# radjkarl/imgProcessor

Hardware: AMD Instinct MI355X
Metric: Mpix/s undistort+5x5 filter, 4K f32 (higher is better)
Workload: dtype f32

## Files before the change

imgprocessor_amd/csrc/fused_sep_c.hip:

```cpp
#include "fused_sep_impl.hpp"

int ipa_fused_sep_launch_c(ipa_ctx* ctx, const ipa::FusedCall& f, const ipa::FusedSep& q) {
  return ipa::fused_sep_k<1>(ctx, f, q);
}

template <typename T> static int strip_remap_int_launch(ipa_ctx* ctx, const ipa::FusedCall& f) {
  using namespace ipa;
  using Src = SampleRowSrc<T, kLinear, MapCoord>;
  FusedCall part[2];
  const SharedPlan plan = fused_plan(ctx, sep_shared<Src, 1>::value && IPA_PIPE_EDGE, f, part);
  if (plan == kPerFrameLoop) return 1;
  if (plan == kSharedLoop) part[0] = f;
  const int parts = plan == kSharedSplit ? 2 : 1;
  for (int i = 0; i < parts; i++) {
    WaveParams p = part[i].p;
    sep_grid<Src, 1>(ctx, p, part[i].n_frames);
    if (!p.frames_wg) return 1;
  }
  Src s;
  fused_source(s, f, f.map);
  s.q5 = 1;
  s.ccval = 0.f;
  const double one = 1.0;
  for (int i = 0; i < parts; i++) {
    s.src = part[i].src;
    const int rc = launch_sep<Src, 1, T>(ctx, part[i].p, s, &one, &one, part[i].n_frames, 0.f);
    if (rc) return rc;
  }
  return IPA_OK;
}
int ipa_fused_sep_launch_c16(ipa_ctx* ctx, const ipa::FusedCall& f) { return strip_remap_int_launch<uint16_t>(ctx, f); }
int ipa_fused_sep_launch_c8(ipa_ctx* ctx, const ipa::FusedCall& f) { return strip_remap_int_launch<uint8_t>(ctx, f); }
```

imgprocessor_amd/csrc/wave_pipe.hpp:

```cpp
#pragma once

namespace ipa {

typedef int v4i __attribute__((ext_vector_type(4)));

#ifndef IPA_PIPE
#define IPA_PIPE 1
#endif
#ifndef IPA_PIPE_ROWS
#define IPA_PIPE_ROWS 4
#endif
#ifndef IPA_PIPE_REUSE
#define IPA_PIPE_REUSE 1
#endif
#ifndef IPA_PIPE_STAY
#define IPA_PIPE_STAY 0
#endif
#ifndef IPA_SHARE_TAPS
#define IPA_SHARE_TAPS 0
#endif
#ifndef IPA_DEBUG_HALO_LEVEL
#define IPA_DEBUG_HALO_LEVEL 0
#endif
#ifndef IPA_LANE_NATURAL
// ... 84 lines not shown
}
__device__ __forceinline__ void pipe_store1(unsigned x, unsigned voff, uint8_t* sbase) {
  asm volatile(IPA_SGPR_HAZARD "global_store_dword %0, %1, %2 " IPA_STORE_FLAVOUR "\n\ts_nop 0" ::"v"(voff), "v"(x), "s"(sbase));
}
__device__ __forceinline__ unsigned cv16_round(float v) {
  float r = rintf(v);
  r = r > 0.f ? r : 0.f;
  r = r < 65535.f ? r : 65535.f;
  return (unsigned)r;
}
__device__ __forceinline__ void pipe_gather2(float& a, float& b, unsigned off, v4i rs) {
#ifdef IPA_DEBUG_NO_GATHER
  a = __uint_as_float(off | 0x3f000000u);
  b = a;
  return;
#endif
#ifdef IPA_DEBUG_ONE_DWORD
  asm volatile(IPA_SGPR_HAZARD "buffer_load_dword %0, %1, %2, 0 offen" : "=v"(a) : "v"(off), "s"(rs));
  b = a;
  return;
#endif
  asm volatile(IPA_SGPR_HAZARD "buffer_load_dword %0, %2, %3, 0 offen\n\t"
               "buffer_load_dword %1, %2, %3, 0 offen offset:4"
               : "=v"(a), "=v"(b)
               : "v"(off), "s"(rs));
}
__device__ __forceinline__ void pipe_gather1(float& a, unsigned off, v4i rs) {
  asm volatile(IPA_SGPR_HAZARD "buffer_load_dword %0, %1, %2, 0 offen" : "=v"(a) : "v"(off), "s"(rs));
}
__device__ __forceinline__ void pipe_gather1_b16(float& a, unsigned off, v4i rs) {
  asm volatile(IPA_SGPR_HAZARD "buffer_load_ushort %0, %1, %2, 0 offen" : "=v"(a) : "v"(off), "s"(rs));
}
__device__ __forceinline__ void pipe_gather1_b16_masked(float& a, unsigned off, v4i rs, unsigned long long m) {
  unsigned long long sv;
  asm volatile(IPA_SGPR_HAZARD "s_mov_b64 %1, exec\n\t"
               "s_mov_b64 exec, %4\n\t"
               "buffer_load_ushort %0, %2, %3, 0 offen\n\t"
               "s_mov_b64 exec, %1"
               : "+v"(a), "=&s"(sv)
               : "v"(off), "s"(rs), "s"(m));
}
__device__ __forceinline__ void pipe_gather1_masked(float& a, unsigned off, v4i rs,
                                                    unsigned long long m) {
  unsigned long long sv;
  asm volatile(IPA_SGPR_HAZARD "s_mov_b64 %1, exec\n\t"
               "s_mov_b64 exec, %4\n\t"
               "buffer_load_dword %0, %2, %3, 0 offen\n\t"
// ... 391 lines not shown
    else vm_wait<kTapOps>();
    pin_map(m);
    footprint(m, txnn, tynn, offnn, interiornn);
    issue_map(m, t + 3);
  };

  float txc[NS], tyc[NS];
  unsigned offc[NS], inc = (1u << NS) - 1u;
  int tb = 0;
#pragma unroll 1
  do {
    if (tb + 0 < T) step(tb + 0, ga, gb, txa, tya, offa, ina, txb, tyb, offb, inb, txc, tyc, offc, inc);
    if (tb + 1 < T) step(tb + 1, gb, ga, txb, tyb, offb, inb, txc, tyc, offc, inc, txa, tya, offa, ina);
    if (tb + 2 < T) step(tb + 2, ga, gb, txc, tyc, offc, inc, txa, tya, offa, ina, txb, tyb, offb, inb);
    if (tb + 3 < T) step(tb + 3, gb, ga, txa, tya, offa, ina, txb, tyb, offb, inb, txc, tyc, offc, inc);
    if (tb + 4 < T) step(tb + 4, ga, gb, txb, tyb, offb, inb, txc, tyc, offc, inc, txa, tya, offa, ina);
    if (tb + 5 < T) step(tb + 5, gb, ga, txc, tyc, offc, inc, txa, tya, offa, ina, txb, tyb, offb, inb);
    tb += 6;
  } while (tb < T);
#undef hoff
}

template <bool HALO> struct ring_row { static constexpr int value = HALO ? 832 + 128 : 832; };

template <int K> struct DenseFilter {
  static constexpr int kTaps = K;
  const Weights<float, K * K>& wts;
  unsigned lane4_opaque;
  v2f acc[K][2];
  __device__ __forceinline__ DenseFilter(const Weights<float, K * K>& w) : wts(w) {
    lane4_opaque = 4u * (threadIdx.x & 63u);
    asm volatile("" : "+v"(lane4_opaque));
  }
  template <bool EDGE> __device__ __forceinline__ v4f row(const float* xp, unsigned lane, const Cols&) {
    return pipe_filter_row<K>(wts, xp, lane, lane4_opaque, acc);
  }
};

template <int K, int QM, bool EDGE, bool HALO, typename Filter, typename ST, typename Coord, bool CV16 = false>
__device__ __forceinline__ void wave_run_strip_shared(const WaveParams& p,
                                                      const SampleRowSrc<ST, kLinear, Coord>& src,
                                                      Filter& filt, float* xp, float* ring,
                                                      unsigned wave, const Cols& c, int y0,
                                                      int nrows, bool writer, float* dst) {
  using G = wave_geom<K, HALO>;
  using C = typename Coord::coord_t;
  constexpr int NS = 4;
  constexpr int NSP = HALO ? 5 : 4;
  constexpr int HP = 2 * G::H;
  static_assert(!HALO || HP <= 8, "at most 8 halo pixels (32 halo lanes, 128 record floats)");
  constexpr int RR = ring_row<HALO>::value;
  constexpr bool kTable = coord_is_table<Coord>::value;
  constexpr int NR = sizeof(ST) == 4 ? 2 : 1;
  constexpr int SH = sizeof(ST) == 4 ? 2 : (sizeof(ST) == 2 ? 1 : 0);
  constexpr bool kU8 = sizeof(ST) == 1;
  constexpr bool FIX8 = kU8 && CV16;
  static_assert(std::is_same<ST, float>::value || std::is_same<ST, uint16_t>::value || std::is_same<ST, uint8_t>::value,
                "float32 / uint16 / uint8 frames");
  constexpr int W = IPA_WPB;
  constexpr bool NAT = IPA_LANE_NATURAL != 0 && !HALO;
  constexpr int R = 2 * W;
  constexpr int kMapOps = kTable ? 2 * NSP : 0;
  static_assert(W == 2 || W == 4 || W == 8, "steps of a block alternate the tap-register roles");
  const int T = nrows + K - 1;
  const unsigned lane = threadIdx.x & 63u;
  constexpr unsigned CB = sizeof(C);
  const unsigned voff = 16u * lane, moff = NAT ? 4u * CB * lane : CB * lane;
  auto ucol = [&](int k) -> int { return NAT ? c.uu[k] : c.uq[k]; };
  auto pxcol = [&](int k) -> int { return NAT ? 4 * (int)lane + k : (int)lane + 64 * k; };
  static_assert(!CV16 || (K == 1 && QM == 1 && !HALO && sizeof(ST) <= 2), "CV16: integer frames, 1/32-px coordinates, no filter");
  float* outs = dst + ((long)y0 * p.dpitch + c.xs);
  uint16_t* outs16 = reinterpret_cast<uint16_t*>(dst) + ((long)y0 * p.dpitch + c.xs);
  uint8_t* outs8 = reinterpret_cast<uint8_t*>(dst) + ((long)y0 * p.dpitch + c.xs);
  const int yb = y0 - G::H;
  const C* mxr = nullptr;
  const C* myr = nullptr;
  if constexpr (kTable) {
    mxr = src.coord.mx + (EDGE ? 0 : (long)yb * src.coord.pitch + c.xs);
    myr = src.coord.my + (EDGE ? 0 : (long)yb * src.coord.pitch + c.xs);
  }
  auto row_of = [&](int t) -> int {
    if constexpr (EDGE) return resolve_idx(yb + t, p.dh, p.cby);
    else return yb + t;
  };
  const SrcView& s = src.s;
  const unsigned long long fb = (unsigned long long)src.fbase;
  const v4i rs = v4i{(int)(unsigned)fb, (int)((unsigned)(fb >> 32) & 0xffffu), (int)src.src_bytes,
                     0x00020000};
  const unsigned pitch_b = (unsigned)s.pitch << SH;
  float* rlane = ring + 4u * lane;
  const unsigned hcol = halo_pos<G::H>(lane);
  const unsigned long long pmask = (1ull << HP) - 1ull;
  const unsigned long long qmask = (1ull << (4 * HP)) - 1ull;
  const unsigned hq = lane < 4u * HP ? lane >> 2 : (unsigned)HP - 1u;
  const unsigned hpos = kRowPad - G::H + halo_pos<G::H>(hq);
  int uhq = 0;
  if constexpr (HALO && EDGE) uhq = resolve_idx(c.xs - G::H + (int)halo_pos<G::H>(hq), p.dw, p.cbx);
  constexpr unsigned kHTapIn = 1u, kHAnyIn = 2u, kHSlow = 4u, kHInterior = 8u;

  C pm[2 * NSP] = {};
  auto issue_coords = [&](int r) {
    if constexpr (kTable) {
      if constexpr (EDGE) {
        const int rr = row_of(r < T ? r : T - 1);
        const long o = (long)(rr < 0 ? 0 : rr) * src.coord.pitch;
#pragma unroll
        for (int k = 0; k < 4; k++) pipe_load1<0>(pm[k], CB * (unsigned)(ucol(k) < 0 ? 0 : ucol(k)), mxr + o);
        if constexpr (HALO) pipe_load1_masked<0>(pm[4], CB * (unsigned)(c.uh < 0 ? 0 : c.uh), mxr + o, pmask);
#pragma unroll
        for (int k = 0; k < 4; k++) pipe_load1<0>(pm[NSP + k], CB * (unsigned)(ucol(k) < 0 ? 0 : ucol(k)), myr + o);
        if constexpr (HALO) pipe_load1_masked<0>(pm[NSP + 4], CB * (unsigned)(c.uh < 0 ? 0 : c.uh), myr + o, pmask);
      } else {
        const long o = (long)(r < T ? r : T - 1) * src.coord.pitch;
        static_for<0, 4>([&](auto Kk) {
          constexpr int k = decltype(Kk)::value;
          pipe_load1<(NAT ? 1 : 64) * (int)CB * k>(pm[k], moff, mxr + o);
        });
        if constexpr (HALO) pipe_load1_masked<0>(pm[4], CB * hcol, mxr + o - G::H, pmask);
        static_for<0, 4>([&](auto Kk) {
          constexpr int k = decltype(Kk)::value;
          pipe_load1<(NAT ? 1 : 64) * (int)CB * k>(pm[NSP + k], moff, myr + o);
        });
        if constexpr (HALO) pipe_load1_masked<0>(pm[NSP + 4], CB * hcol, myr + o - G::H, pmask);
      }
    }
  };
  auto publish = [&](int r) {
    C sx[NSP], sy[NSP];
    if constexpr (kTable) {
#pragma unroll
      for (int k = 0; k < 2 * NSP; k++) vm_pin(pm[k]);
#pragma unroll
      for (int k = 0; k < NSP; k++) { sx[k] = pm[k]; sy[k] = pm[NSP + k]; }
    } else {
      const int rc = r < T ? r : T - 1;
      const int rr = row_of(rc);
#pragma unroll
      for (int k = 0; k < 4; k++) {
        if constexpr (EDGE) src.coord.get(ucol(k) < 0 ? 0 : ucol(k), rr < 0 ? 0 : rr, sx[k], sy[k]);
        else src.coord.get(c.xs + pxcol(k), rr, sx[k], sy[k]);
      }
      if constexpr (HALO) {
        if constexpr (EDGE) src.coord.get(c.uh < 0 ? 0 : c.uh, rr < 0 ? 0 : rr, sx[4], sy[4]);
        else src.coord.get(c.xs - G::H + (int)(lane < (unsigned)HP ? hcol : (unsigned)G::H), rr, sx[4], sy[4]);
      }
    }
    float tx[NSP], ty[NSP];
    int e[NSP];
    unsigned interior;
    batch_footprint_linear<NSP, QM>(s, sx, sy, tx, ty, e, interior);
    if constexpr (HALO) interior |= lane < (unsigned)HP ? 0u : 0x10u;
    if (s.border == IPA_BORDER_CONSTANT && __builtin_amdgcn_ballot_w64(interior != (1u << NSP) - 1u))
      interior |= border_tap_bits<NSP, QM, NR == 1, C>(s, sx, sy, interior);
    float* slot = rlane + (unsigned)(r % R) * RR;
    *reinterpret_cast<v4i*>(slot) = v4i{e[0] << SH, e[1] << SH, e[2] << SH, e[3] << SH};
    *reinterpret_cast<v4f*>(slot + 256) = v4f{tx[0], tx[1], tx[2], tx[3]};
    *reinterpret_cast<v4f*>(slot + 512) = v4f{ty[0], ty[1], ty[2], ty[3]};
    float* rowp = ring + (unsigned)(r % R) * RR;
    reinterpret_cast<unsigned*>(rowp + 768)[lane] = interior & ~0x0f000010u;
    if constexpr (HALO) {
      if (lane < (unsigned)HP) {
        const bool in4 = (interior >> 4) & 1u;
        const unsigned vb = (interior >> 24) & 15u;
        const bool slow = !in4 && (s.border != IPA_BORDER_CONSTANT || (interior & kBorderSlow) != 0u);
        float* hrow = rowp + 832 + 16u * lane;
#pragma unroll
        for (int tap = 0; tap < 4; tap++) {
          const unsigned o = ((unsigned)e[4] << SH) + (NR == 2 ? (unsigned)(tap & 1) * 4u : 0u) +
                             (unsigned)(tap >> 1) * pitch_b;
          const unsigned fl = ((in4 || ((vb >> tap) & 1u)) ? kHTapIn : 0u) | ((in4 || vb) ? kHAnyIn : 0u) |
                              (slow ? kHSlow : 0u) | (in4 ? kHInterior : 0u);
          *reinterpret_cast<v4f*>(hrow + 4 * tap) = v4f{__uint_as_float(o), tx[4], ty[4], __uint_as_float(fl)};
        }
      }
    }
  };
  auto footprint = [&](int r, float (&tx)[NS], float (&ty)[NS], unsigned (&off)[NS],
                       unsigned& interior) {
    const float* slot = rlane + (unsigned)(r % R) * RR;
    const float* rowp = ring + (unsigned)(r % R) * RR;
    const v4i qo = *reinterpret_cast<const v4i*>(slot);
    const v4f qx = *reinterpret_cast<const v4f*>(slot + 256), qy = *reinterpret_cast<const v4f*>(slot + 512);
    interior = reinterpret_cast<const unsigned*>(rowp + 768)[lane];
    off[0] = (unsigned)qo.x; off[1] = (unsigned)qo.y; off[2] = (unsigned)qo.z; off[3] = (unsigned)qo.w;
    tx[0] = qx.x; tx[1] = qx.y; tx[2] = qx.z; tx[3] = qx.w;
    ty[0] = qy.x; ty[1] = qy.y; ty[2] = qy.z; ty[3] = qy.w;
  };
  auto halo_record = [&](int r, unsigned& off, float& tx, float& ty, unsigned& fl) {
    const float* rowp = ring + (unsigned)(r % R) * RR;
    const v4f q = *reinterpret_cast<const v4f*>(rowp + 832 + 4u * (lane < 4u * HP ? lane : 4u * HP - 1u));
    off = __float_as_uint(q.x); tx = q.y; ty = q.z; fl = __float_as_uint(q.w);
  };
  auto gather = [&](float (&g)[NS * NR], int k, unsigned o) {
#if IPA_SHARE_TAPS == 9
    if constexpr (NR == 2) { pipe_gather1(g[2 * k], o, rs); return; }
#endif
    if constexpr (NR == 2) pipe_gather2(g[2 * k], g[2 * k + 1], o, rs);
    else if constexpr (kU8) pipe_gather1_b16(g[k], o, rs);
    else pipe_gather1(g[k], o, rs);
  };
  auto gather_masked = [&](float (&g)[NS * NR], int k, unsigned o, unsigned long long m) {
#if IPA_SHARE_TAPS == 9
    if constexpr (NR == 2) { pipe_gather1_masked(g[2 * k], o, rs, m); return; }
#endif
    if constexpr (NR == 2) pipe_gather2_masked(g[2 * k], g[2 * k + 1], o, rs, m);
    else if constexpr (kU8) pipe_gather1_b16_masked(g[k], o, rs, m);
    else pipe_gather1_masked(g[k], o, rs, m);
// ... 11 lines not shown
#if IPA_SHARE_TAPS == 9
    if constexpr (NR == 2) { v0 = g[2 * k]; v1 = from_lane_above(v0); return; }
#endif
    if constexpr (NR == 2) { v0 = g[2 * k]; v1 = g[2 * k + 1]; }
    else if constexpr (kU8) { v0 = (float)(__float_as_uint(g[k]) & 0xffu); v1 = (float)((__float_as_uint(g[k]) >> 8) & 0xffu); }
    else TapLoad<uint16_t, float>::unpack(__float_as_uint(g[k]), v0, v1);
  };

  float ga[NS * NR] = {}, gb[NS * NR] = {};
  float txa[NS], tya[NS], txb[NS], tyb[NS];
  unsigned offa[NS], offb[NS], ina, inb;
  float hga = 0.f, hgb = 0.f, htxa = 0.f, htya = 0.f, htxb = 0.f, htyb = 0.f;
  unsigned hfla = 0u, hflb = 0u;

#ifdef IPA_DEBUG_STAMPS
  unsigned stamp_acc[8] = {0, 0, 0, 0, 0, 0, 0, 0};
  unsigned stamp_prev = 0;
#define IPA_STAMP0() stamp_prev = (unsigned)__builtin_amdgcn_s_memtime()
#define IPA_STAMP(i) { const unsigned now_ = (unsigned)__builtin_amdgcn_s_memtime(); stamp_acc[i] += now_ - stamp_prev; stamp_prev = now_; }
#else
#define IPA_STAMP0()
#define IPA_STAMP(i)
#endif
  issue_coords((int)wave);
  vm_wait<0>();
  publish((int)wave);
  asm volatile("s_waitcnt lgkmcnt(0)\n\ts_barrier" ::: "memory");
  issue_coords(W + (int)wave);
  footprint(0, txa, tya, offa, ina);
  gather_row(ga, offa, 0u);
  gather_row(gb, offa, pitch_b);
  if constexpr (HALO && IPA_DEBUG_HALO_LEVEL < 2) {
    unsigned ho;
    halo_record(0, ho, htxa, htya, hfla);
    if (IPA_DEBUG_HALO_LEVEL < 1) pipe_gather1_masked(hga, ho, rs, qmask);
  }

  auto step = [&](auto St, int t, float (&top)[NS * NR], float (&bot)[NS * NR], const float (&tx)[NS],
                  const float (&ty)[NS], const unsigned (&off)[NS], unsigned interior,
                  float (&txn)[NS], float (&tyn)[NS], unsigned (&offn)[NS], unsigned& interiorn,
                  float& hg, float htx, float hty, unsigned hfl,
                  float& hgn, float& htxn, float& htyn, unsigned& hfln) {
    constexpr int STEP = decltype(St)::value;
    IPA_STAMP0();
    if constexpr (STEP == W - 1) {
#ifndef IPA_DEBUG_NO_BARRIER
      asm volatile("s_waitcnt lgkmcnt(0)\n\ts_barrier" ::: "memory");
#endif
      IPA_STAMP(0);
      issue_coords(t + 1 + W + (int)wave);
    }
    const bool stored = t >= K && t <= T;
    if constexpr (STEP == W - 1) {
      if (stored) vm_wait<kMapOps + 1>();
      else vm_wait<kMapOps>();
    } else {
      if (stored) vm_wait<1>();
      else vm_wait<0>();
    }
    pin_taps(top);
    pin_taps(bot);
    IPA_STAMP(1);
    if constexpr (HALO && IPA_DEBUG_HALO_LEVEL < 1) vm_pin(hg);
    if constexpr (STEP == W - 2) publish(t + 2 + (int)wave);
    float cur[NS];
#pragma unroll
    for (int k = 0; k < NS; k++) {
      const float wx0 = 1.f - tx[k], wx1 = tx[k], wy0 = 1.f - ty[k], wy1 = ty[k];
      float v00, v01, v10, v11;
      taps_of(top, k, v00, v01);
      taps_of(bot, k, v10, v11);
      if constexpr (FIX8) {
        cur[k] = fix8_sum((int)v00, (int)v01, (int)v10, (int)v11, tx[k], ty[k]);
      } else if constexpr (CV16) {
        cur[k] = cv16_sum(v00, v01, v10, v11, wx0, wx1, wy0, wy1);
      } else {
        float r0 = wx0 * v00;
        r0 = ipa_fma(wx1, v01, r0);
        float o = wy0 * r0;
        float r1 = wx0 * v10;
        r1 = ipa_fma(wx1, v11, r1);
        cur[k] = ipa_fma(wy1, r1, o);
      }
    }
    int rowt = 0;
    if constexpr (EDGE) {
      rowt = row_of(t < T ? t : T - 1);
#pragma unroll
      for (int k = 0; k < 4; k++) cur[k] = (rowt < 0 || ucol(k) < 0) ? src.ccval : cur[k];
    }
    if constexpr (NAT) {
      *reinterpret_cast<v4f*>(xp + kRowPad + 4u * lane) = v4f{cur[0], cur[1], cur[2], cur[3]};
    } else {
#pragma unroll
      for (int k = 0; k < 4; k++) xp[kRowPad + 64u * k + lane] = cur[k];
    }
    if constexpr (HALO && IPA_DEBUG_HALO_LEVEL < 2) {
      float v = hg;
      if constexpr (NR == 1) {
        float lo, hi;
        TapLoad<uint16_t, float>::unpack(__float_as_uint(hg), lo, hi);
        v = (lane & 1u) ? hi : lo;
      }
      v = (hfl & kHTapIn) ? v : src.cval;
      const int vi = __float_as_int(v);
      const float v00 = __int_as_float(__builtin_amdgcn_update_dpp(vi, vi, 0x00, 0xf, 0xf, false));
      const float v01 = __int_as_float(__builtin_amdgcn_update_dpp(vi, vi, 0x55, 0xf, 0xf, false));
      const float v10 = __int_as_float(__builtin_amdgcn_update_dpp(vi, vi, 0xaa, 0xf, 0xf, false));
      const float v11 = __int_as_float(__builtin_amdgcn_update_dpp(vi, vi, 0xff, 0xf, 0xf, false));
      const float wx0 = 1.f - htx, wx1 = htx, wy0 = 1.f - hty, wy1 = hty;
      float r0 = wx0 * v00;
      r0 = ipa_fma(wx1, v01, r0);
// ... 18 lines not shown
      if (__builtin_amdgcn_ballot_w64(interior != (1u << NS) - 1u)) {
#pragma unroll
        for (int k = 0; k < NS; k++) {
          if (!((interior >> k) & 1u) && !(interior & kBorderSlow)) {
            float v00, v01, v10, v11;
            taps_of(top, k, v00, v01);
            taps_of(bot, k, v10, v11);
            float o;
            if constexpr (FIX8) {
              const unsigned vb = (interior >> (8 + 4 * k)) & 15u;
              const int cv = (int)src.cval;
              o = fix8_sum((vb & 1u) ? (int)v00 : cv, (vb & 2u) ? (int)v01 : cv, (vb & 4u) ? (int)v10 : cv,
                           (vb & 8u) ? (int)v11 : cv, tx[k], ty[k]);
              o = vb ? o : src.cval;
            } else if constexpr (CV16) {
              const unsigned vb = (interior >> (8 + 4 * k)) & 15u;
              o = cv16_sum((vb & 1u) ? v00 : src.cval, (vb & 2u) ? v01 : src.cval, (vb & 4u) ? v10 : src.cval,
                           (vb & 8u) ? v11 : src.cval, 1.f - tx[k], tx[k], 1.f - ty[k], ty[k]);
              o = vb ? o : src.cval;
            } else {
              o = border_blend(v00, v01, v10, v11, tx[k], ty[k], (interior >> (8 + 4 * k)) & 15u, src.cval);
            }
            bool keep = true;
            if constexpr (EDGE) keep = !(rowt < 0 || ucol(k) < 0);
            if (keep) xp[kRowPad + (unsigned)pxcol(k)] = o;
          }
        }
      }
    }
    if (__builtin_amdgcn_ballot_w64(s.border == IPA_BORDER_CONSTANT ? (interior & kBorderSlow) != 0u
                                                                     : interior != (1u << NS) - 1u)) {
#pragma unroll 1
      for (int k = 0; k < NS; k++) {
        if (!((interior >> k) & 1u) && (s.border != IPA_BORDER_CONSTANT || (interior & kBorderSlow))) {
          C sx, sy;
          const int col = c.xs + pxcol(k);
          const unsigned pos = kRowPad + (unsigned)pxcol(k);
          if constexpr (EDGE) {
            const int uqk = resolve_idx(col, p.dw, p.cbx);
            src.coord.get(uqk < 0 ? 0 : uqk, rowt < 0 ? 0 : rowt, sx, sy);
            if (!(rowt < 0 || uqk < 0)) {
              if constexpr (FIX8) xp[pos] = (float)sample_u8_fixed<C>(s, sx, sy, (uint8_t)src.cval);
              else if constexpr (CV16) xp[pos] = (float)sample_u16_cv<kLinear, C>(s, nullptr, sx, sy, (uint16_t)src.cval);
              else xp[pos] = sample<ST, kLinear, C>(s, sx, sy, src.cval);
            }
          } else {
            src.coord.get(col, yb + (t < T ? t : T - 1), sx, sy);
// ... 19 lines not shown
      if (__builtin_amdgcn_ballot_w64(stay)) {
#pragma unroll
        for (int j = 0; j < NR; j++) bot[NR * k + j] = stay ? top[NR * k + j] : bot[NR * k + j];
      }
      unsigned long long need =
          __builtin_amdgcn_ballot_w64(offn[k] != off[k] + pitch_b && !stay);
      if (need) gather_masked(bot, k, offn[k], need);
#else
      gather(bot, k, offn[k]);
#endif
    }
    gather_row(top, offn, pitch_b);
    if constexpr (HALO && IPA_DEBUG_HALO_LEVEL < 2) {
      unsigned ho;
      halo_record(t + 1 < T ? t + 1 : T - 1, ho, htxn, htyn, hfln);
      if (IPA_DEBUG_HALO_LEVEL < 1) pipe_gather1_masked(hgn, ho, rs, qmask);
      else hgn = __uint_as_float(ho | 0x3f000000u);
    }
    __builtin_amdgcn_wave_barrier();
    IPA_STAMP(3);
#ifdef IPA_DEBUG_NO_FILTER
    const v4f q = *reinterpret_cast<const v4f*>(xp + kRowPad + 4u * lane);
#else
    const v4f q = filt.template row<EDGE>(xp, lane, c);
#endif
    const int o = t - (K - 1);
#ifdef IPA_DEBUG_STAMPS
    { float qx = q.x; asm volatile("" : "+v"(qx)); }
#endif
    IPA_STAMP(4);
    if (o >= 0 && o < nrows) {
      if constexpr (FIX8) {
        const unsigned px = (unsigned)q.x | ((unsigned)q.y << 8) | ((unsigned)q.z << 16) | ((unsigned)q.w << 24);
        if (writer) pipe_store1(px, 4u * lane, outs8 + (long)o * p.dpitch);
      } else if constexpr (CV16) {
        const unsigned lo = cv16_round(q.x) | (cv16_round(q.y) << 16), hi = cv16_round(q.z) | (cv16_round(q.w) << 16);
        if (writer) pipe_store2(lo, hi, 8u * lane, outs16 + (long)o * p.dpitch);
      } else {
        if (writer) pipe_store4<true>(q, voff, outs + (long)o * p.dpitch);
      }
    }
    __builtin_amdgcn_wave_barrier();
    IPA_STAMP(5);
#ifdef IPA_DEBUG_STAMPS
    stamp_acc[7] += 1;
#endif
  };
// ... 29 lines not shown
```

imgprocessor_amd/csrc/wave_sep.hpp:

```cpp
#pragma once

#include "common.hpp"
#include "wave_stencil.hpp"

namespace ipa {

#ifndef IPA_SEP_MIN_HL
#define IPA_SEP_MIN_HL 2
#endif
template <int K> struct sep_geom {
  static constexpr int HL = (K / 2 + 3) / 4 > IPA_SEP_MIN_HL ? (K / 2 + 3) / 4 : IPA_SEP_MIN_HL;
  static constexpr int OW = 256 - 8 * HL;
};
template <> struct sep_geom<1> {
  static constexpr int HL = 0;
  static constexpr int OW = 256;
};

template <int K> struct SepTaps {
  float ky[K], kx[K];
};

template <typename Src, int K> struct sep_depth {
  static constexpr int value = Src::kMap ? Src::template depth<K>::value : 1;
// ... 143 lines not shown
        }
        if (writer) {
          float* row = dst + (long)(y0 + o) * p.dpitch + c.xo;
          const int n = p.dw - c.xo < 4 ? p.dw - c.xo : 4;
          if constexpr (FAST) {
            float* rows_ = dst + ((long)(y0 + o) * p.dpitch + c.xs);
            *reinterpret_cast<float4*>(rows_ + 4u * (threadIdx.x & 63u)) =
                float4{out[0], out[1], out[2], out[3]};
          } else if (p.vec_out && n == 4) {
            *reinterpret_cast<float4*>(row) = float4{out[0], out[1], out[2], out[3]};
          } else {
#pragma unroll
            for (int k = 0; k < 4; k++)
              if (k < n) row[k] = out[k];
          }
        }
      }
    });
    if constexpr (!kRegs) __builtin_amdgcn_wave_barrier();
  }
}

template <int K> struct SepFilter {
  const SepTaps<K>& w;
  float xcval;
  float acc[K][4];
  v2f acc2[K][2];
  __device__ __forceinline__ SepFilter(const SepTaps<K>& taps, float xc) : w(taps), xcval(xc) {}
  template <bool EDGE> __device__ __forceinline__ v4f row(const float* xp, unsigned lane, const Cols& c) {
    constexpr int H = K / 2;
    const float4 q = *reinterpret_cast<const float4*>(xp + kRowPad + 4u * lane);
    const float cur[4] = {q.x, q.y, q.z, q.w};
    if constexpr (IPA_SEP_PACKED != 0) {
      sep_y_pass<K>(w, acc2, v2f{cur[0], cur[1]}, v2f{cur[2], cur[3]});
      float mid[4] = {acc2[K - 1][0].x, acc2[K - 1][0].y, acc2[K - 1][1].x, acc2[K - 1][1].y};
      if constexpr (EDGE) {
#pragma unroll
        for (int k = 0; k < 4; k++)
          if (c.uu[k] < 0) mid[k] = xcval;
      }
      return sep_x_pass<K>(w, mid);
    }
    static_for<0, K>([&](auto Ii) {
      constexpr int i = K - 1 - decltype(Ii)::value;
#pragma unroll
      for (int ox = 0; ox < 4; ox++) {
        if constexpr (i == 0) acc[0][ox] = w.ky[0] * cur[ox];
        else acc[i][ox] = fmaf(w.ky[i], cur[ox], acc[i - 1][ox]);
      }
    });
    float mid[4];
#pragma unroll
    for (int k = 0; k < 4; k++) mid[k] = acc[K - 1][k];
    if constexpr (EDGE) {
#pragma unroll
      for (int k = 0; k < 4; k++)
        if (c.uu[k] < 0) mid[k] = xcval;
    }
    float win[4 + 2 * H];
#pragma unroll
    for (int k = 0; k < 4; k++) win[H + k] = mid[k];
#pragma unroll
    for (int m = 0; m < H; m++) {
      win[H - 1 - m] = from_lane_below(mid[3 - m]);
      win[H + 4 + m] = from_lane_above(mid[m]);
    }
    float out[4];
#pragma unroll
    for (int ox = 0; ox < 4; ox++) {
      float a = w.kx[0] * win[ox];
#pragma unroll
      for (int j = 1; j < K; j++) a = fmaf(w.kx[j], win[ox + j], a);
      out[ox] = a;
    }
    return v4f{out[0], out[1], out[2], out[3]};
  }
};

template <typename Src, int K> struct sep_shared : std::false_type {};
template <typename ST, typename Coord, int K> struct sep_shared<SampleRowSrc<ST, kLinear, Coord>, K> {
  static constexpr bool value = IPA_PIPE != 0 && IPA_PIPE_SHARED != 0 &&
                                (std::is_same<ST, float>::value || std::is_same<ST, uint16_t>::value ||
                                 std::is_same<ST, uint8_t>::value);
};

template <typename Src> struct sep_shares_maps : std::false_type {};
template <typename ST, int I, typename Coord>
struct sep_shares_maps<SampleRowSrc<ST, I, Coord>> {
  static constexpr bool value = coord_is_table<Coord>::value ||
                                (I == kLinear && IPA_PIPE != 0 && IPA_PIPE_SHARED != 0);
};

template <typename Src, int K, typename DT = float>
__global__ void __launch_bounds__(256)
wave_sep_kernel(WaveParams p, Src src, SepTaps<K> w, float xcval) {
  constexpr bool kCv16 = std::is_same<DT, uint16_t>::value || std::is_same<DT, uint8_t>::value;
  static_assert(std::is_same<DT, float>::value || (kCv16 && K == 1), "float32 results, or the integer strip remaps");
  constexpr int H = K / 2, D = sep_depth<Src, K>::value, HL = sep_geom<K>::HL, OW = sep_geom<K>::OW;
  constexpr bool kRegs = std::is_same<Src, LoadRowSrc>::value;
  __shared__ __attribute__((aligned(16))) float xpose[kRegs ? 1 : 4 * kRowStride * D];
  static_assert(H <= 4 * HL, "the halo lanes hold the x pass's neighbours");
  const int lane = threadIdx.x & 63;
  unsigned b = xcd_swizzle(blockIdx.x, gridDim.x), frame = blockIdx.y;
  if (p.frame_major) {
    frame = b / p.frame_major;
    b -= frame * p.frame_major;
  } else if (p.frames_inner) {
    frame = b % (unsigned)p.frames_inner;
    b /= (unsigned)p.frames_inner;
  }
  const unsigned wave = __builtin_amdgcn_readfirstlane(threadIdx.x >> 6);
  unsigned sid = b * 4 + wave;
  if (p.frames_wg) {
    const unsigned groups = (unsigned)p.frames_inner / 4u;
    b = xcd_swizzle(blockIdx.x, gridDim.x);
    if (p.group_chunk) {
      const unsigned gc = (unsigned)p.group_chunk, per = gc * p.strips;
      const unsigned chunk = b / per, r = b - chunk * per;
      frame = (chunk * gc + r % gc) * 4u + wave;
      sid = r / gc;
    } else {
      frame = (b % groups) * 4u + wave;
      sid = b / groups;
    }
  }
  float* xp = xpose + (kRegs ? 0 : wave * kRowStride * D);
  constexpr bool kShared = sep_shared<Src, K>::value;
  __shared__ __attribute__((aligned(16))) float mapring[kShared ? 2 * 4 * ring_row<false>::value : 4];
  static_assert(!kShared || IPA_WPB == 4, "the separable kernel runs 4 waves per workgroup");
  if (sid >= p.strips) return;
  const int syi = (int)(sid / (unsigned)p.strips_x), sxi = (int)sid - syi * p.strips_x;
  src.set_frame(frame);
  const int xs = sxi * OW - 4 * HL;
  Cols c;
  c.xs = xs;
  c.xo = xs + lane * 4;
  int y0, nrows;
  if (!wave_strip_rows(p, syi, y0, nrows)) return;
  const bool writer = lane >= HL && lane < 64 - HL && c.xo < p.dw;
  float* dst = reinterpret_cast<float*>(reinterpret_cast<DT*>(p.dst) + (long)frame * p.dst_frame_elems);
  const int rows_touched = ((nrows + K - 1 + D - 1) / D) * D;
  const bool fast = !p.no_pipe && src.vectors_ok() && p.vec_out && xs >= 0 && xs + 256 <= p.dw &&
                    y0 - H >= 0 && y0 - H + rows_touched <= p.dh;
  if (fast) {
#pragma unroll
    for (int k = 0; k < 4; k++) c.uu[k] = c.xo + k;
    if constexpr (kShared) {
      if (p.frames_wg) {
        SepFilter<K> filt(w, xcval);
        if constexpr (kCv16) {
          wave_run_strip_shared<K, 1, false, false, SepFilter<K>, typename Src::sample_type, typename Src::coord_type, true>(
              p, src, filt, xp, mapring, wave, c, y0, nrows, writer, dst);
        } else {
          if (src.q5) wave_run_strip_shared<K, 1, false, false>(p, src, filt, xp, mapring, wave, c, y0, nrows, writer, dst);
          else wave_run_strip_shared<K, 0, false, false>(p, src, filt, xp, mapring, wave, c, y0, nrows, writer, dst);
        }
        return;
      }
    }
    if constexpr (kCv16) return;
    else if constexpr (!kRegs) {
      if (src.q5) wave_sep_strip<true, Src, K, 1>(p, src, w, xp, c, y0, nrows, writer, dst, xcval);
      else wave_sep_strip<true, Src, K, 0>(p, src, w, xp, c, y0, nrows, writer, dst, xcval);
    } else {
      wave_sep_strip<true, Src, K>(p, src, w, xp, c, y0, nrows, writer, dst, xcval);
    }
  } else {
#pragma unroll
    for (int k = 0; k < 4; k++) {
      c.uu[k] = resolve_idx(c.xo + k, p.dw, p.cbx);
      c.uq[k] = resolve_idx(xs + lane + 64 * k, p.dw, p.cbx);
    }
    if constexpr (kShared) {
      if (p.frames_wg && !p.no_pipe && src.vectors_ok() && p.vec_out && (p.dw & 3) == 0 && IPA_PIPE_EDGE) {
        SepFilter<K> filt(w, xcval);
        if constexpr (kCv16) {
          wave_run_strip_shared<K, 1, true, false, SepFilter<K>, typename Src::sample_type, typename Src::coord_type, true>(
              p, src, filt, xp, mapring, wave, c, y0, nrows, writer, dst);
        } else {
          if (src.q5) wave_run_strip_shared<K, 1, true, false>(p, src, filt, xp, mapring, wave, c, y0, nrows, writer, dst);
          else wave_run_strip_shared<K, 0, true, false>(p, src, filt, xp, mapring, wave, c, y0, nrows, writer, dst);
        }
        return;
      }
    }
    if constexpr (!kCv16) wave_sep_strip<false, Src, K>(p, src, w, xp, c, y0, nrows, writer, dst, xcval);
  }
}

template <typename Src, int K> static dim3 sep_grid(ipa_ctx* ctx, WaveParams& p, int n_frames) {
  const bool shared_run = shared_loop_plan(ctx, sep_shared<Src, K>::value, n_frames, true) == kSharedLoop;
  wave_strips(ctx, p, sep_geom<K>::OW, n_frames, K, false,
              shared_run ? 2 : (std::is_same<Src, LoadRowSrc>::value ? 1 : 0));
  return wave_grid(ctx, p, n_frames, 4, true, sep_shares_maps<Src>::value, std::is_same<Src, LoadRowSrc>::value, -K);
}

template <typename Src, int K, typename DT = float>
static int launch_sep(ipa_ctx* ctx, WaveParams p, const Src& src, const double* ky,
                      const double* kx, int n_frames, float xcval) {
  SepTaps<K> w;
  for (int i = 0; i < K; i++) {
    w.ky[i] = (float)ky[i];
    w.kx[i] = (float)kx[i];
  }
  const dim3 grid = sep_grid<Src, K>(ctx, p, n_frames);
  hipLaunchKernelGGL((wave_sep_kernel<Src, K, DT>), grid, dim3(256), 0, ctx->stream, p, src, w, xcval);
  IPA_HIP(ctx, hipGetLastError());
  return IPA_OK;
}

}
```

imgprocessor_amd/csrc/wave_stencil.hpp:

```cpp
#pragma once

#include <type_traits>

#include "common.hpp"
#include "conv_tile.hpp"
#include "sampler.hpp"

#ifndef IPA_PIPE
#define IPA_PIPE 1
#endif
#ifndef IPA_PIPE_MAX_K
#define IPA_PIPE_MAX_K 7
#endif
#ifndef IPA_PIPE_MIN_WAVES
#define IPA_PIPE_MIN_WAVES 4
#endif
#ifndef IPA_WPB
#define IPA_WPB 4
#endif
#ifndef IPA_PIPE_EDGE
#define IPA_PIPE_EDGE 1
#endif
#ifndef IPA_PIPE_SHARED
#define IPA_PIPE_SHARED 1
// ... 259 lines not shown
  };

  Coord coord;
  const char* src;
  long src_frame_bytes;
  unsigned src_bytes;
  int sh, sw, spitch;
  int border, q5;
  float cubic_a;
  const float* lanczos;
  float cval;
  float ccval;
  int map_vec;
  SrcView s;
  const char* fbase;

  __device__ __forceinline__ void set_frame(unsigned f) {
    fbase = src + (long)f * src_frame_bytes;
    s.rsrc = make_rsrc(fbase, src_bytes);
    s.h = sh; s.w = sw; s.pitch = spitch;
    s.border = border; s.q5 = q5; s.cubic_a = cubic_a; s.lanczos = lanczos;
    s.pair_split = 1;
  }
  __device__ __forceinline__ bool vectors_ok() const { return !kMap || map_vec != 0; }

  template <bool FAST>
  __device__ __forceinline__ void coords_of_row(const Cols& c, int vv, C (&sx)[4],
                                                C (&sy)[4]) const {
    const int lane = threadIdx.x & 63;
#pragma unroll
    for (int k = 0; k < 4; k++) {
      if constexpr (FAST) coord.get(c.xs + lane + 64 * k, vv, sx[k], sy[k]);
      else coord.get(c.uq[k] < 0 ? 0 : c.uq[k], vv < 0 ? 0 : vv, sx[k], sy[k]);
    }
  }

  static constexpr bool kHasQ5 = true;
  template <bool FAST, int D, int QM = -1>
  __device__ __forceinline__ void load_chunk(const Cols& c, const int (&vv)[D],
                                             Chunk<D>& ch) const {
    C sx[D][4], sy[D][4];
    if constexpr (kMap && FAST) {
      const unsigned lane = threadIdx.x & 63u;
#pragma unroll
      for (int d = 0; d < D; d++) {
        const long o = (long)vv[d] * coord.pitch + c.xs;
        const float* rx = coord.mx + o;
// ... 459 lines not shown
```

Before: 551,900.

## Add lean shared-loop separable kernel variant with register-pressure reductions

Splits the separable wave kernel into a dedicated LEAN instantiation for the shared-record loop, chosen on the host, and requests 5 waves per EU through amdgpu_waves_per_eu. Register pressure is reduced several ways: column-index data is packed into bitmasks or read back from LDS, interpolation fractions are loaded late from the ring, and an early-clobber constraint is added on the gather asm. The aim is higher occupancy and less branching over the non-shared paths. The cost is extra LDS reads and LDS space per step, and possible spills under the tighter register budget.

```diff
diff --git a/imgprocessor_amd/csrc/fused_sep_c.hip b/imgprocessor_amd/csrc/fused_sep_c.hip
--- a/imgprocessor_amd/csrc/fused_sep_c.hip
+++ b/imgprocessor_amd/csrc/fused_sep_c.hip
@@ -12,15 +12,15 @@
   if (plan == kPerFrameLoop) return 1;
   if (plan == kSharedLoop) part[0] = f;
   const int parts = plan == kSharedSplit ? 2 : 1;
-  for (int i = 0; i < parts; i++) {
-    WaveParams p = part[i].p;
-    sep_grid<Src, 1>(ctx, p, part[i].n_frames);
-    if (!p.frames_wg) return 1;
-  }
   Src s;
   fused_source(s, f, f.map);
   s.q5 = 1;
   s.ccval = 0.f;
+  for (int i = 0; i < parts; i++) {
+    WaveParams p = part[i].p;
+    sep_grid<Src, 1>(ctx, p, part[i].n_frames);
+    if (!sep_lean_launch<Src, 1>(p, s)) return 1;
+  }
   const double one = 1.0;
   for (int i = 0; i < parts; i++) {
     s.src = part[i].src;
diff --git a/imgprocessor_amd/csrc/wave_pipe.hpp b/imgprocessor_amd/csrc/wave_pipe.hpp
--- a/imgprocessor_amd/csrc/wave_pipe.hpp
+++ b/imgprocessor_amd/csrc/wave_pipe.hpp
@@ -130,7 +130,7 @@
 #endif
   asm volatile(IPA_SGPR_HAZARD "buffer_load_dword %0, %2, %3, 0 offen\n\t"
                "buffer_load_dword %1, %2, %3, 0 offen offset:4"
-               : "=v"(a), "=v"(b)
+               : "=&v"(a), "=v"(b)
                : "v"(off), "s"(rs));
 }
 __device__ __forceinline__ void pipe_gather1(float& a, unsigned off, v4i rs) {
@@ -568,9 +568,11 @@
 }
 
 template <bool HALO> struct ring_row { static constexpr int value = HALO ? 832 + 128 : 832; };
+constexpr int kRingCols = 256;
 
 template <int K> struct DenseFilter {
   static constexpr int kTaps = K;
+  static constexpr bool kTightRegisters = false;
   const Weights<float, K * K>& wts;
   unsigned lane4_opaque;
   v2f acc[K][2];
@@ -578,7 +580,7 @@
     lane4_opaque = 4u * (threadIdx.x & 63u);
     asm volatile("" : "+v"(lane4_opaque));
   }
-  template <bool EDGE> __device__ __forceinline__ v4f row(const float* xp, unsigned lane, const Cols&) {
+  template <bool EDGE> __device__ __forceinline__ v4f row(const float* xp, unsigned lane, unsigned) {
     return pipe_filter_row<K>(wts, xp, lane, lane4_opaque, acc);
   }
 };
@@ -607,12 +609,35 @@
   constexpr bool NAT = IPA_LANE_NATURAL != 0 && !HALO;
   constexpr int R = 2 * W;
   constexpr int kMapOps = kTable ? 2 * NSP : 0;
+  constexpr bool LATE = Filter::kTightRegisters && !HALO;
   static_assert(W == 2 || W == 4 || W == 8, "steps of a block alternate the tap-register roles");
   const int T = nrows + K - 1;
   const unsigned lane = threadIdx.x & 63u;
   constexpr unsigned CB = sizeof(C);
   const unsigned voff = 16u * lane, moff = NAT ? 4u * CB * lane : CB * lane;
-  auto ucol = [&](int k) -> int { return NAT ? c.uu[k] : c.uq[k]; };
+  constexpr bool LDSCOL = EDGE && Filter::kTightRegisters && !HALO && !NAT;
+  unsigned cbits = 0u;
+  if constexpr (EDGE && Filter::kTightRegisters) {
+#pragma unroll
+    for (int k = 0; k < 4; k++) cbits |= ((NAT ? c.uu[k] : c.uq[k]) < 0 ? 1u << k : 0u) | (c.uu[k] < 0 ? 16u << k : 0u);
+  }
+  int* colword = reinterpret_cast<int*>(ring + R * RR) + 4u * lane;
+  if constexpr (LDSCOL) {
+    if (wave == 0) *reinterpret_cast<v4i*>(colword) = v4i{c.uq[0], c.uq[1], c.uq[2], c.uq[3]};
+  }
+  auto ucols = [&](int (&u)[4], auto first) {
+    if constexpr (LDSCOL && !decltype(first)::value) {
+      const v4i q = *reinterpret_cast<const v4i*>(colword);
+      u[0] = q.x; u[1] = q.y; u[2] = q.z; u[3] = q.w;
+    } else {
+#pragma unroll
+      for (int k = 0; k < 4; k++) u[k] = NAT ? c.uu[k] : c.uq[k];
+    }
+  };
+  auto ucol_const = [&](int k) -> bool {
+    if constexpr (Filter::kTightRegisters) return (cbits >> k) & 1u;
+    else return (NAT ? c.uu[k] : c.uq[k]) < 0;
+  };
   auto pxcol = [&](int k) -> int { return NAT ? 4 * (int)lane + k : (int)lane + 64 * k; };
   static_assert(!CV16 || (K == 1 && QM == 1 && !HALO && sizeof(ST) <= 2), "CV16: integer frames, 1/32-px coordinates, no filter");
   float* outs = dst + ((long)y0 * p.dpitch + c.xs);
@@ -645,16 +670,18 @@
   constexpr unsigned kHTapIn = 1u, kHAnyIn = 2u, kHSlow = 4u, kHInterior = 8u;
 
   C pm[2 * NSP] = {};
-  auto issue_coords = [&](int r) {
+  auto issue_coords = [&](int r, auto first) {
     if constexpr (kTable) {
       if constexpr (EDGE) {
         const int rr = row_of(r < T ? r : T - 1);
         const long o = (long)(rr < 0 ? 0 : rr) * src.coord.pitch;
-#pragma unroll
-        for (int k = 0; k < 4; k++) pipe_load1<0>(pm[k], CB * (unsigned)(ucol(k) < 0 ? 0 : ucol(k)), mxr + o);
+        int uc[4];
+        ucols(uc, first);
+#pragma unroll
+        for (int k = 0; k < 4; k++) pipe_load1<0>(pm[k], CB * (unsigned)(uc[k] < 0 ? 0 : uc[k]), mxr + o);
         if constexpr (HALO) pipe_load1_masked<0>(pm[4], CB * (unsigned)(c.uh < 0 ? 0 : c.uh), mxr + o, pmask);
 #pragma unroll
-        for (int k = 0; k < 4; k++) pipe_load1<0>(pm[NSP + k], CB * (unsigned)(ucol(k) < 0 ? 0 : ucol(k)), myr + o);
+        for (int k = 0; k < 4; k++) pipe_load1<0>(pm[NSP + k], CB * (unsigned)(uc[k] < 0 ? 0 : uc[k]), myr + o);
         if constexpr (HALO) pipe_load1_masked<0>(pm[NSP + 4], CB * (unsigned)(c.uh < 0 ? 0 : c.uh), myr + o, pmask);
       } else {
         const long o = (long)(r < T ? r : T - 1) * src.coord.pitch;
@@ -671,7 +698,7 @@
       }
     }
   };
-  auto publish = [&](int r) {
+  auto publish = [&](int r, auto first) {
     C sx[NSP], sy[NSP];
     if constexpr (kTable) {
 #pragma unroll
@@ -681,9 +708,11 @@
     } else {
       const int rc = r < T ? r : T - 1;
       const int rr = row_of(rc);
+      int uc[4] = {0, 0, 0, 0};
+      if constexpr (EDGE) ucols(uc, first);
 #pragma unroll
       for (int k = 0; k < 4; k++) {
-        if constexpr (EDGE) src.coord.get(ucol(k) < 0 ? 0 : ucol(k), rr < 0 ? 0 : rr, sx[k], sy[k]);
+        if constexpr (EDGE) src.coord.get(uc[k] < 0 ? 0 : uc[k], rr < 0 ? 0 : rr, sx[k], sy[k]);
         else src.coord.get(c.xs + pxcol(k), rr, sx[k], sy[k]);
       }
       if constexpr (HALO) {
@@ -726,9 +755,17 @@
     const float* slot = rlane + (unsigned)(r % R) * RR;
     const float* rowp = ring + (unsigned)(r % R) * RR;
     const v4i qo = *reinterpret_cast<const v4i*>(slot);
-    const v4f qx = *reinterpret_cast<const v4f*>(slot + 256), qy = *reinterpret_cast<const v4f*>(slot + 512);
     interior = reinterpret_cast<const unsigned*>(rowp + 768)[lane];
     off[0] = (unsigned)qo.x; off[1] = (unsigned)qo.y; off[2] = (unsigned)qo.z; off[3] = (unsigned)qo.w;
+    if constexpr (!LATE) {
+      const v4f qx = *reinterpret_cast<const v4f*>(slot + 256), qy = *reinterpret_cast<const v4f*>(slot + 512);
+      tx[0] = qx.x; tx[1] = qx.y; tx[2] = qx.z; tx[3] = qx.w;
+      ty[0] = qy.x; ty[1] = qy.y; ty[2] = qy.z; ty[3] = qy.w;
+    }
+  };
+  auto fractions = [&](int r, float (&tx)[NS], float (&ty)[NS]) {
+    const float* slot = rlane + (unsigned)(r % R) * RR;
+    const v4f qx = *reinterpret_cast<const v4f*>(slot + 256), qy = *reinterpret_cast<const v4f*>(slot + 512);
     tx[0] = qx.x; tx[1] = qx.y; tx[2] = qx.z; tx[3] = qx.w;
     ty[0] = qy.x; ty[1] = qy.y; ty[2] = qy.z; ty[3] = qy.w;
   };
@@ -786,11 +823,11 @@
 #define IPA_STAMP0()
 #define IPA_STAMP(i)
 #endif
-  issue_coords((int)wave);
+  issue_coords((int)wave, std::true_type{});
   vm_wait<0>();
-  publish((int)wave);
+  publish((int)wave, std::true_type{});
   asm volatile("s_waitcnt lgkmcnt(0)\n\ts_barrier" ::: "memory");
-  issue_coords(W + (int)wave);
+  issue_coords(W + (int)wave, std::false_type{});
   footprint(0, txa, tya, offa, ina);
   gather_row(ga, offa, 0u);
   gather_row(gb, offa, pitch_b);
@@ -800,19 +837,26 @@
     if (IPA_DEBUG_HALO_LEVEL < 1) pipe_gather1_masked(hga, ho, rs, qmask);
   }
 
-  auto step = [&](auto St, int t, float (&top)[NS * NR], float (&bot)[NS * NR], const float (&tx)[NS],
-                  const float (&ty)[NS], const unsigned (&off)[NS], unsigned interior,
+  auto step = [&](auto St, int t, float (&top)[NS * NR], float (&bot)[NS * NR], const float (&txr)[NS],
+                  const float (&tyr)[NS], const unsigned (&off)[NS], unsigned interior,
                   float (&txn)[NS], float (&tyn)[NS], unsigned (&offn)[NS], unsigned& interiorn,
                   float& hg, float htx, float hty, unsigned hfl,
                   float& hgn, float& htxn, float& htyn, unsigned& hfln) {
     constexpr int STEP = decltype(St)::value;
     IPA_STAMP0();
+    float tx[NS], ty[NS];
+    if constexpr (LATE) {
+      if constexpr (STEP != W - 2) fractions(t < T ? t : T - 1, tx, ty);
+    } else {
+#pragma unroll
+      for (int k = 0; k < NS; k++) { tx[k] = txr[k]; ty[k] = tyr[k]; }
+    }
     if constexpr (STEP == W - 1) {
 #ifndef IPA_DEBUG_NO_BARRIER
       asm volatile("s_waitcnt lgkmcnt(0)\n\ts_barrier" ::: "memory");
 #endif
       IPA_STAMP(0);
-      issue_coords(t + 1 + W + (int)wave);
+      issue_coords(t + 1 + W + (int)wave, std::false_type{});
     }
     const bool stored = t >= K && t <= T;
     if constexpr (STEP == W - 1) {
@@ -826,7 +870,8 @@
     pin_taps(bot);
     IPA_STAMP(1);
     if constexpr (HALO && IPA_DEBUG_HALO_LEVEL < 1) vm_pin(hg);
-    if constexpr (STEP == W - 2) publish(t + 2 + (int)wave);
+    if constexpr (STEP == W - 2) publish(t + 2 + (int)wave, std::false_type{});
+    if constexpr (LATE && STEP == W - 2) fractions(t < T ? t : T - 1, tx, ty);
     float cur[NS];
 #pragma unroll
     for (int k = 0; k < NS; k++) {
@@ -851,7 +896,7 @@
     if constexpr (EDGE) {
       rowt = row_of(t < T ? t : T - 1);
 #pragma unroll
-      for (int k = 0; k < 4; k++) cur[k] = (rowt < 0 || ucol(k) < 0) ? src.ccval : cur[k];
+      for (int k = 0; k < 4; k++) cur[k] = (rowt < 0 || ucol_const(k)) ? src.ccval : cur[k];
     }
     if constexpr (NAT) {
       *reinterpret_cast<v4f*>(xp + kRowPad + 4u * lane) = v4f{cur[0], cur[1], cur[2], cur[3]};
@@ -916,7 +961,7 @@
               o = border_blend(v00, v01, v10, v11, tx[k], ty[k], (interior >> (8 + 4 * k)) & 15u, src.cval);
             }
             bool keep = true;
-            if constexpr (EDGE) keep = !(rowt < 0 || ucol(k) < 0);
+            if constexpr (EDGE) keep = !(rowt < 0 || ucol_const(k));
             if (keep) xp[kRowPad + (unsigned)pxcol(k)] = o;
           }
         }
@@ -982,7 +1027,7 @@
 #ifdef IPA_DEBUG_NO_FILTER
     const v4f q = *reinterpret_cast<const v4f*>(xp + kRowPad + 4u * lane);
 #else
-    const v4f q = filt.template row<EDGE>(xp, lane, c);
+    const v4f q = filt.template row<EDGE>(xp, lane, cbits >> 4);
 #endif
     const int o = t - (K - 1);
 #ifdef IPA_DEBUG_STAMPS
diff --git a/imgprocessor_amd/csrc/wave_sep.hpp b/imgprocessor_amd/csrc/wave_sep.hpp
--- a/imgprocessor_amd/csrc/wave_sep.hpp
+++ b/imgprocessor_amd/csrc/wave_sep.hpp
@@ -189,12 +189,13 @@
 }
 
 template <int K> struct SepFilter {
+  static constexpr bool kTightRegisters = true;
   const SepTaps<K>& w;
   float xcval;
   float acc[K][4];
   v2f acc2[K][2];
   __device__ __forceinline__ SepFilter(const SepTaps<K>& taps, float xc) : w(taps), xcval(xc) {}
-  template <bool EDGE> __device__ __forceinline__ v4f row(const float* xp, unsigned lane, const Cols& c) {
+  template <bool EDGE> __device__ __forceinline__ v4f row(const float* xp, unsigned lane, unsigned xconst) {
     constexpr int H = K / 2;
     const float4 q = *reinterpret_cast<const float4*>(xp + kRowPad + 4u * lane);
     const float cur[4] = {q.x, q.y, q.z, q.w};
@@ -204,7 +205,7 @@
       if constexpr (EDGE) {
 #pragma unroll
         for (int k = 0; k < 4; k++)
-          if (c.uu[k] < 0) mid[k] = xcval;
+          if ((xconst >> k) & 1u) mid[k] = xcval;
       }
       return sep_x_pass<K>(w, mid);
     }
@@ -222,7 +223,7 @@
     if constexpr (EDGE) {
 #pragma unroll
       for (int k = 0; k < 4; k++)
-        if (c.uu[k] < 0) mid[k] = xcval;
+        if ((xconst >> k) & 1u) mid[k] = xcval;
     }
     float win[4 + 2 * H];
 #pragma unroll
@@ -258,43 +259,53 @@
                                 (I == kLinear && IPA_PIPE != 0 && IPA_PIPE_SHARED != 0);
 };
 
-template <typename Src, int K, typename DT = float>
-__global__ void __launch_bounds__(256)
+#ifndef IPA_SEP_LEAN_WAVES
+#define IPA_SEP_LEAN_WAVES 5
+#endif
+template <typename Src, int K, bool LEAN> struct sep_lean_waves { static constexpr int value = 1; };
+template <typename ST, int K> struct sep_lean_waves<SampleRowSrc<ST, kLinear, MapCoord>, K, true> {
+  static constexpr int value = K <= 5 ? IPA_SEP_LEAN_WAVES : 1;
+};
+
+template <typename Src, int K, typename DT = float, bool LEAN = false, int QM = 0>
+__global__ void __launch_bounds__(256) __attribute__((amdgpu_waves_per_eu(sep_lean_waves<Src, K, LEAN>::value)))
 wave_sep_kernel(WaveParams p, Src src, SepTaps<K> w, float xcval) {
   constexpr bool kCv16 = std::is_same<DT, uint16_t>::value || std::is_same<DT, uint8_t>::value;
   static_assert(std::is_same<DT, float>::value || (kCv16 && K == 1), "float32 results, or the integer strip remaps");
+  static_assert(!kCv16 || LEAN, "integer results are written on the shared-record loop alone");
+  static_assert(!LEAN || (sep_shared<Src, K>::value && IPA_PIPE_EDGE), "the lean form is the shared-record loop");
+  static_assert(!LEAN || IPA_WPB == 4, "the separable kernel runs 4 waves per workgroup");
   constexpr int H = K / 2, D = sep_depth<Src, K>::value, HL = sep_geom<K>::HL, OW = sep_geom<K>::OW;
   constexpr bool kRegs = std::is_same<Src, LoadRowSrc>::value;
   __shared__ __attribute__((aligned(16))) float xpose[kRegs ? 1 : 4 * kRowStride * D];
+  __shared__ __attribute__((aligned(16))) float mapring[(LEAN ? 2 * 4 * ring_row<false>::value + kRingCols : 4) + IPA_DEBUG_LDS_PAD];
   static_assert(H <= 4 * HL, "the halo lanes hold the x pass's neighbours");
   const int lane = threadIdx.x & 63;
   unsigned b = xcd_swizzle(blockIdx.x, gridDim.x), frame = blockIdx.y;
-  if (p.frame_major) {
-    frame = b / p.frame_major;
-    b -= frame * p.frame_major;
-  } else if (p.frames_inner) {
-    frame = b % (unsigned)p.frames_inner;
-    b /= (unsigned)p.frames_inner;
-  }
   const unsigned wave = __builtin_amdgcn_readfirstlane(threadIdx.x >> 6);
-  unsigned sid = b * 4 + wave;
-  if (p.frames_wg) {
-    const unsigned groups = (unsigned)p.frames_inner / 4u;
-    b = xcd_swizzle(blockIdx.x, gridDim.x);
+  unsigned sid;
+  if (LEAN || p.frames_wg) {
     if (p.group_chunk) {
       const unsigned gc = (unsigned)p.group_chunk, per = gc * p.strips;
       const unsigned chunk = b / per, r = b - chunk * per;
       frame = (chunk * gc + r % gc) * 4u + wave;
       sid = r / gc;
     } else {
+      const unsigned groups = (unsigned)p.frames_inner / 4u;
       frame = (b % groups) * 4u + wave;
       sid = b / groups;
     }
+  } else {
+    if (p.frame_major) {
+      frame = b / p.frame_major;
+      b -= frame * p.frame_major;
+    } else if (p.frames_inner) {
+      frame = b % (unsigned)p.frames_inner;
+      b /= (unsigned)p.frames_inner;
+    }
+    sid = b * 4 + wave;
   }
   float* xp = xpose + (kRegs ? 0 : wave * kRowStride * D);
-  constexpr bool kShared = sep_shared<Src, K>::value;
-  __shared__ __attribute__((aligned(16))) float mapring[kShared ? 2 * 4 * ring_row<false>::value : 4];
-  static_assert(!kShared || IPA_WPB == 4, "the separable kernel runs 4 waves per workgroup");
   if (sid >= p.strips) return;
   const int syi = (int)(sid / (unsigned)p.strips_x), sxi = (int)sid - syi * p.strips_x;
   src.set_frame(frame);
@@ -307,52 +318,54 @@
   const bool writer = lane >= HL && lane < 64 - HL && c.xo < p.dw;
   float* dst = reinterpret_cast<float*>(reinterpret_cast<DT*>(p.dst) + (long)frame * p.dst_frame_elems);
   const int rows_touched = ((nrows + K - 1 + D - 1) / D) * D;
-  const bool fast = !p.no_pipe && src.vectors_ok() && p.vec_out && xs >= 0 && xs + 256 <= p.dw &&
-                    y0 - H >= 0 && y0 - H + rows_touched <= p.dh;
-  if (fast) {
-#pragma unroll
-    for (int k = 0; k < 4; k++) c.uu[k] = c.xo + k;
-    if constexpr (kShared) {
-      if (p.frames_wg) {
-        SepFilter<K> filt(w, xcval);
-        if constexpr (kCv16) {
-          wave_run_strip_shared<K, 1, false, false, SepFilter<K>, typename Src::sample_type, typename Src::coord_type, true>(
-              p, src, filt, xp, mapring, wave, c, y0, nrows, writer, dst);
-        } else {
-          if (src.q5) wave_run_strip_shared<K, 1, false, false>(p, src, filt, xp, mapring, wave, c, y0, nrows, writer, dst);
-          else wave_run_strip_shared<K, 0, false, false>(p, src, filt, xp, mapring, wave, c, y0, nrows, writer, dst);
-        }
-        return;
-      }
-    }
-    if constexpr (kCv16) return;
-    else if constexpr (!kRegs) {
-      if (src.q5) wave_sep_strip<true, Src, K, 1>(p, src, w, xp, c, y0, nrows, writer, dst, xcval);
-      else wave_sep_strip<true, Src, K, 0>(p, src, w, xp, c, y0, nrows, writer, dst, xcval);
+  const bool inside = xs >= 0 && xs + 256 <= p.dw && y0 - H >= 0 && y0 - H + rows_touched <= p.dh;
+  if constexpr (LEAN) {
+    SepFilter<K> filt(w, xcval);
+#ifdef IPA_DEBUG_LEAN_ONLY
+    if (IPA_DEBUG_LEAN_ONLY == 1) {
+#else
+    if (inside) {
+#endif
+#pragma unroll
+      for (int k = 0; k < 4; k++) c.uu[k] = c.xo + k;
+      wave_run_strip_shared<K, QM, false, false, SepFilter<K>, typename Src::sample_type, typename Src::coord_type, kCv16>(
+          p, src, filt, xp, mapring, wave, c, y0, nrows, writer, dst);
     } else {
-      wave_sep_strip<true, Src, K>(p, src, w, xp, c, y0, nrows, writer, dst, xcval);
+#pragma unroll
+      for (int k = 0; k < 4; k++) {
+        c.uu[k] = resolve_idx(c.xo + k, p.dw, p.cbx);
+        c.uq[k] = resolve_idx(xs + lane + 64 * k, p.dw, p.cbx);
+      }
+      wave_run_strip_shared<K, QM, true, false, SepFilter<K>, typename Src::sample_type, typename Src::coord_type, kCv16>(
+          p, src, filt, xp, mapring, wave, c, y0, nrows, writer, dst);
     }
   } else {
-#pragma unroll
-    for (int k = 0; k < 4; k++) {
-      c.uu[k] = resolve_idx(c.xo + k, p.dw, p.cbx);
-      c.uq[k] = resolve_idx(xs + lane + 64 * k, p.dw, p.cbx);
-    }
-    if constexpr (kShared) {
-      if (p.frames_wg && !p.no_pipe && src.vectors_ok() && p.vec_out && (p.dw & 3) == 0 && IPA_PIPE_EDGE) {
-        SepFilter<K> filt(w, xcval);
-        if constexpr (kCv16) {
-          wave_run_strip_shared<K, 1, true, false, SepFilter<K>, typename Src::sample_type, typename Src::coord_type, true>(
-              p, src, filt, xp, mapring, wave, c, y0, nrows, writer, dst);
-        } else {
-          if (src.q5) wave_run_strip_shared<K, 1, true, false>(p, src, filt, xp, mapring, wave, c, y0, nrows, writer, dst);
-          else wave_run_strip_shared<K, 0, true, false>(p, src, filt, xp, mapring, wave, c, y0, nrows, writer, dst);
-        }
-        return;
-      }
-    }
-    if constexpr (!kCv16) wave_sep_strip<false, Src, K>(p, src, w, xp, c, y0, nrows, writer, dst, xcval);
-  }
+    (void)mapring;
+    if (!p.no_pipe && src.vectors_ok() && p.vec_out && inside) {
+#pragma unroll
+      for (int k = 0; k < 4; k++) c.uu[k] = c.xo + k;
+      if constexpr (!kRegs) {
+        if (src.q5) wave_sep_strip<true, Src, K, 1>(p, src, w, xp, c, y0, nrows, writer, dst, xcval);
+        else wave_sep_strip<true, Src, K, 0>(p, src, w, xp, c, y0, nrows, writer, dst, xcval);
+      } else {
+        wave_sep_strip<true, Src, K>(p, src, w, xp, c, y0, nrows, writer, dst, xcval);
+      }
+    } else {
+#pragma unroll
+      for (int k = 0; k < 4; k++) {
+        c.uu[k] = resolve_idx(c.xo + k, p.dw, p.cbx);
+        c.uq[k] = resolve_idx(xs + lane + 64 * k, p.dw, p.cbx);
+      }
+      wave_sep_strip<false, Src, K>(p, src, w, xp, c, y0, nrows, writer, dst, xcval);
+    }
+  }
+}
+
+template <typename Src, int K> static bool sep_lean_launch(const WaveParams& p, const Src& src) {
+  if constexpr (sep_shared<Src, K>::value && IPA_PIPE_EDGE)
+    return p.frames_wg && !p.no_pipe && src.vectors_ok() && p.vec_out && (p.dw & 3) == 0;
+  else
+    return false;
 }
 
 template <typename Src, int K> static dim3 sep_grid(ipa_ctx* ctx, WaveParams& p, int n_frames) {
@@ -371,9 +384,23 @@
     w.kx[i] = (float)kx[i];
   }
   const dim3 grid = sep_grid<Src, K>(ctx, p, n_frames);
-  hipLaunchKernelGGL((wave_sep_kernel<Src, K, DT>), grid, dim3(256), 0, ctx->stream, p, src, w, xcval);
-  IPA_HIP(ctx, hipGetLastError());
-  return IPA_OK;
-}
-
-}
+  if constexpr (sep_shared<Src, K>::value && IPA_PIPE_EDGE) {
+    if (sep_lean_launch<Src, K>(p, src)) {
+      if (src.q5 || !std::is_same<DT, float>::value)
+        hipLaunchKernelGGL((wave_sep_kernel<Src, K, DT, true, 1>), grid, dim3(256), 0, ctx->stream, p, src, w, xcval);
+      else if constexpr (std::is_same<DT, float>::value)
+        hipLaunchKernelGGL((wave_sep_kernel<Src, K, DT, true, 0>), grid, dim3(256), 0, ctx->stream, p, src, w, xcval);
+      IPA_HIP(ctx, hipGetLastError());
+      return IPA_OK;
+    }
+  }
+  if constexpr (std::is_same<DT, float>::value) {
+    hipLaunchKernelGGL((wave_sep_kernel<Src, K, DT>), grid, dim3(256), 0, ctx->stream, p, src, w, xcval);
+    IPA_HIP(ctx, hipGetLastError());
+    return IPA_OK;
+  } else {
+    return 1;
+  }
+}
+
+}
diff --git a/imgprocessor_amd/csrc/wave_stencil.hpp b/imgprocessor_amd/csrc/wave_stencil.hpp
--- a/imgprocessor_amd/csrc/wave_stencil.hpp
+++ b/imgprocessor_amd/csrc/wave_stencil.hpp
@@ -305,7 +305,7 @@
     s.border = border; s.q5 = q5; s.cubic_a = cubic_a; s.lanczos = lanczos;
     s.pair_split = 1;
   }
-  __device__ __forceinline__ bool vectors_ok() const { return !kMap || map_vec != 0; }
+  __host__ __device__ __forceinline__ bool vectors_ok() const { return !kMap || map_vec != 0; }
 
   template <bool FAST>
   __device__ __forceinline__ void coords_of_row(const Cols& c, int vv, C (&sx)[4],
```

Result: no change. 556,400 (median of 6 runs) (+0.8%).
